# oliverhu/rama

Hardware: AMD Instinct MI355X
Metric: tokens/sec decode + matvec achieved-HBM-GB/s vs roofline, llama2-7B fp32 1xMI355X (higher is better)
Workload: dtype f32

## Files before the change

rama_amd/csrc/chain.hpp:

```cpp
#pragma once
#define RAMA_CHAIN_HPP 1
#include "kernels.hpp"
#include "chain_params.hpp"
#include "ref_order.hpp"
#include "topp_sort.hpp"
#include "seqsum_fast.hpp"
#include "handoff.hpp"

namespace rama {


template <int NW>
struct SeqSumShared {
    Inc w[2][NW];
    int ev[2][NW];
    int pos[2];
    float cum[2];
};

template <int R, int NW>
__device__ __forceinline__ void seqsum_round(const float* a, int n, SeqSumShared<NW>& sh, int par) {
    RAMA_NO_CONTRACT
    const int tid = threadIdx.x, lane = tid & 63, wave = tid >> 6;
    const int pos = sh.pos[par];
// ... 328 lines not shown
    float v[R];
#pragma unroll
    for (int k = 0; k < R; k++) { const int i = (int)threadIdx.x * R + k; const float t = a[scan_slot(min(i, n - 1))]; v[k] = i < n ? t : 0.0f; }
    const int nreal = min(max((n - (int)threadIdx.x * R + 7) >> 3, 0), R / 8);
    return seq_sum_fast<NW, R>(v, fs, out, nreal);
}
template <int NW>
__device__ __forceinline__ bool seq_sum_lds_fast(const float* a, int n, FastSumShared<NW>& fs, float* out) {
    const int per = (n + 64 * NW - 1) / (64 * NW);
    if (n < kFastSumMin || per > 64) return false;
    seq_sum_fast_prepare<NW>(fs);
    if (per <= 8) return seq_sum_lds_fast_r<NW, 8>(a, n, fs, out);
    if (per <= 16) return seq_sum_lds_fast_r<NW, 16>(a, n, fs, out);
    if (per <= 32) return seq_sum_lds_fast_r<NW, 32>(a, n, fs, out);
    return seq_sum_lds_fast_r<NW, 64>(a, n, fs, out);
}
template <int NW>
__device__ __forceinline__ float seq_sum_cascade(const float* a, int n, FastSumShared<NW>& fsn, PredShared<NW>& ps, SeqSumShared<NW>& sh) {
    float sum;
    if (!seq_sum_lds_fast<NW>(a, n, fsn, &sum)) { __syncthreads(); if (!seq_sum_predict<NW>(a, n, ps, &sum)) sum = seq_sum_exact<NW>(a, n, sh); }
    return sum;
}
__global__ __launch_bounds__(kNormThreads) void rmsnorm_chain_kernel(float* o, const float* x, const float* w, int n, float* copy_to, int stride = 0) {
    RAMA_NO_CONTRACT
    o += (size_t)blockIdx.x * stride; x += (size_t)blockIdx.x * stride;
    extern __shared__ __attribute__((aligned(16))) float s_sq[];
    __shared__ SeqSumShared<kNormWaves> sh;
    __shared__ PredShared<kNormWaves> ps;
    __shared__ FastSumShared<kNormWaves> fsn;
    const int tid = threadIdx.x;
    SEQ_STAMP(0);
    const bool vec = n % 4 == 0 && ((((uintptr_t)x | (uintptr_t)w | (uintptr_t)o | (uintptr_t)copy_to) & 15) == 0) && n <= 16 * kNormThreads;
    if (vec) {
        const int n4 = n >> 2;
        f4 xv[4], wv[4];
#pragma unroll
        for (int k = 0; k < 4; k++) xv[k] = reinterpret_cast<const f4*>(x)[min(tid + kNormThreads * k, n4 - 1)];
#pragma unroll
        for (int k = 0; k < 4; k++) wv[k] = reinterpret_cast<const f4*>(w)[min(tid + kNormThreads * k, n4 - 1)];
#pragma unroll
        for (int k = 0; k < 4; k++) {
            const int i = tid + kNormThreads * k;
            if (i < n4) {
                float* d = s_sq + scan_slot(4 * i);
                d[0] = xv[k].x * xv[k].x; d[1] = xv[k].y * xv[k].y; d[2] = xv[k].z * xv[k].z; d[3] = xv[k].w * xv[k].w;
            }
        }
        __syncthreads();
        float ss;
        if (!seq_sum_lds_fast<kNormWaves>(s_sq, n, fsn, &ss)) { __syncthreads(); if (!seq_sum_predict<kNormWaves>(s_sq, n, ps, &ss)) ss = seq_sum_exact<kNormWaves>(s_sq, n, sh); }
        const float v = 1.0f / sqrtf(ss / (float)n + 1e-5f);
#pragma unroll
        for (int k = 0; k < 4; k++) {
            const int i = tid + kNormThreads * k;
            if (i < n4) {
                if (copy_to) reinterpret_cast<f4*>(copy_to)[i] = xv[k];
                f4 r;
                r.x = wv[k].x * (v * xv[k].x); r.y = wv[k].y * (v * xv[k].y); r.z = wv[k].z * (v * xv[k].z); r.w = wv[k].w * (v * xv[k].w);
                reinterpret_cast<f4*>(o)[i] = r;
            }
        }
        SEQ_STAMP(6);
        return;
    }
    for (int i = tid; i < n; i += kNormThreads) { const float a = x[i]; s_sq[scan_slot(i)] = a * a; }
    __syncthreads();
    float ss;
    if (!seq_sum_lds_fast<kNormWaves>(s_sq, n, fsn, &ss)) { __syncthreads(); if (!seq_sum_predict<kNormWaves>(s_sq, n, ps, &ss)) ss = seq_sum_exact<kNormWaves>(s_sq, n, sh); }
    const float v = 1.0f / sqrtf(ss / (float)n + 1e-5f);
    for (int i = tid; i < n; i += kNormThreads) {
        const float a = x[i];
        if (copy_to) copy_to[i] = a;
        o[i] = w[i] * (v * a);
    }
}

__global__ __launch_bounds__(kNormThreads) void softmax_chain_kernel(float* x, int n) {
    RAMA_NO_CONTRACT
    extern __shared__ __attribute__((aligned(16))) float s_e[];
    __shared__ SeqSumShared<kNormWaves> sh;
    __shared__ PredShared<kNormWaves> ps;
    __shared__ FastSumShared<kNormWaves> fsn;
    __shared__ float red[16];
    __shared__ unsigned long long s_tab[32];
    const int tid = threadIdx.x;
    exp_tab_fill(s_tab);
    float mx = -INFINITY;
    for (int i = tid; i < n; i += kNormThreads) mx = fmaxf(mx, x[i]);
    mx = block_max(mx, red);
    for (int i = tid; i < n; i += kNormThreads) s_e[scan_slot(i)] = expf_glibc_tab(x[i] - mx, s_tab);
    __syncthreads();
    const float sum = seq_sum_cascade<kNormWaves>(s_e, n, fsn, ps, sh);
    for (int i = tid; i < n; i += kNormThreads) x[i] = s_e[scan_slot(i)] / sum;
}


__device__ __forceinline__ __amdgpu_buffer_rsrc_t make_rsrc_uniform(const void* p, unsigned bytes) {
    const unsigned long long b = (unsigned long long)(uintptr_t)p;
    const unsigned lo = __builtin_amdgcn_readfirstlane((unsigned)b), hi = __builtin_amdgcn_readfirstlane((unsigned)(b >> 32));
    return make_rsrc(reinterpret_cast<const void*>((uintptr_t)(((unsigned long long)hi << 32) | lo)), (unsigned)__builtin_amdgcn_readfirstlane((int)bytes));
}
__device__ __forceinline__ f4 ld_nt_s(__amdgpu_buffer_rsrc_t r, unsigned voff, unsigned soff) {
    return __builtin_bit_cast(f4, __builtin_amdgcn_raw_buffer_load_b128(r, (int)voff, (int)soff, 2));
}

#ifdef RAMA_CHAIN_STAMPS
__device__ unsigned long long g_chain_stamps[64];
__device__ unsigned long long g_chain_all[3 * 4096];
#define CHAIN_STAMP(id) do { if (threadIdx.x == 0) { const unsigned long long t_ = __builtin_amdgcn_s_memrealtime(); \
        if (blockIdx.x == RAMA_CHAIN_STAMP_BLOCK) g_chain_stamps[id] = t_; \
        if (blockIdx.x < 4096 && ((id) == 0 || (id) == 2 || (id) == 4)) g_chain_all[3 * blockIdx.x + (id) / 2] = t_; } } while (0)
#else
#define CHAIN_STAMP(id) do { } while (0)
#endif

constexpr unsigned long long kLeadErr = 0x3100ull;
template <int W, int D, int XD, int EPI, int NORM = CNORM_NONE, int LR = 64>
__device__ __forceinline__ void gemv_chain_body(const ChainParams p, int bid_in) {
    RAMA_NO_CONTRACT
    CHAIN_STAMP(0);
    static_assert(D % XD == 0, "the x ring must divide the weight ring");
    extern __shared__ __attribute__((aligned(16))) float xs[];
    __shared__ float relay[64];
    constexpr int WL = W;
    const int lane = threadIdx.x & 63;
    const int wave_all = WL == 1 ? 0 : __builtin_amdgcn_readfirstlane(threadIdx.x >> 6);
    const int wave = wave_all;
    const int j = lane & 3, rr = lane >> 2;
    const int groups = (p.rows + 15) >> 4;
    if constexpr (NORM == CNORM_LEAD) {
        if (bid_in == 0) {
#ifndef RAMA_LEAD_SOLO
#define RAMA_LEAD_SOLO 1
#endif
            constexpr bool SOLO = RAMA_LEAD_SOLO && WL > 1 && LR * WL <= 64;
            constexpr int WD = SOLO ? 1 : WL, LD = SOLO ? LR * WL : LR;
            if (SOLO && wave_all != 0) return;
            FastSumShared<WD>& fs = *reinterpret_cast<FastSumShared<WD>*>(xs);
#ifdef RAMA_CHAIN_STAMPS
            if (threadIdx.x == 0) g_chain_stamps[40] = __builtin_amdgcn_s_memrealtime();
#endif
            const unsigned ep = *p.epoch;
            const __amdgpu_buffer_rsrc_t rxl = make_rsrc_uniform(p.x, (unsigned)p.K * 4u);
            seq_sum_fast_prepare<WD>(fs);
            float a[LD];
#pragma unroll
            for (int u = 0; u < LD / 4; u++) {
                const f4 xv = ld_c(rxl, ((unsigned)threadIdx.x * (unsigned)LD + 4u * (unsigned)u) * 4u);
                a[4 * u] = xv.x * xv.x; a[4 * u + 1] = xv.y * xv.y; a[4 * u + 2] = xv.z * xv.z; a[4 * u + 3] = xv.w * xv.w;
            }
#ifdef RAMA_CHAIN_STAMPS
            { float t_ = 0.0f;
#pragma unroll
              for (int k = 0; k < LD; k++) t_ += a[k];
              asm volatile("" :: "v"(t_)); }
            if (threadIdx.x == 0) g_chain_stamps[41] = __builtin_amdgcn_s_memrealtime();
#endif
            float ss;
            if (!seq_sum_fast<WD, LD>(a, fs, &ss)) {
                __syncthreads();
#pragma unroll
                for (int k = 0; k < LD; k++) { const int i = (int)threadIdx.x * LD + k; if (i < p.K) xs[i] = a[k]; }
                __syncthreads();
                if (threadIdx.x == 0) { float s_ = 0.0f; for (int i = 0; i < p.K; i++) s_ = s_ + xs[i]; xs[p.K] = s_; }
                __syncthreads();
                ss = xs[p.K];
            }
            const float v = 1.0f / sqrtf(ss / (float)p.K + 1e-5f);
            if (threadIdx.x == 0) put_tagged(p.lead, v, ep);
#ifdef RAMA_CHAIN_STAMPS
            if (threadIdx.x == 0) g_chain_stamps[42] = __builtin_amdgcn_s_memrealtime();
#endif
            if (p.xout) {
                for (int i = threadIdx.x; i < p.K; i += WD * 64) p.xout[i] = p.nw[i] * (v * p.x[i]);
            }
            return;
        }
    }
    const int bid = NORM == CNORM_LEAD ? bid_in - 1 : bid_in;
    int half = -1, bid_g = bid;
    if (W == 1 && p.half_from > 0 && bid >= p.half_from) { half = (bid - p.half_from) & 1; bid_g = p.half_from + ((bid - p.half_from) >> 1); }
    const int m = __builtin_amdgcn_readfirstlane(bid_g / groups), g = __builtin_amdgcn_readfirstlane(bid_g - m * groups);
    const float* Wm = m == 0 ? p.w[0] : (m == 1 ? p.w[1] : p.w[2]);
    const int nblk = p.K >> 4;
    const int nchunk = (nblk + D - 1) / D;
    const bool lane_ok = half < 0 || lane < 32;
    const unsigned lane16 = half < 0 ? (unsigned)lane * 16u : (lane < 32 ? (unsigned)half * 512u + (unsigned)lane * 16u : kOOB);
    static_assert(D % 16 == 0, "a chunk is made of whole 16-block stretches");
    const int n16 = (nblk + 15) >> 4;
    auto stretch = [&](int q) {
        const int left = min(max(nblk - q * 16, 0), 16);
        return make_rsrc_uniform(Wm + ((size_t)g * (size_t)nblk + (size_t)min(q, n16) * 16) * 256, (unsigned)left * 1024u);
    };
    unsigned vo[4];
#pragma unroll
    for (int k = 0; k < 4; k++) vo[k] = lane16 + (unsigned)k * 4096u;
    const __amdgpu_buffer_rsrc_t rx = make_rsrc_uniform(p.x, (unsigned)p.K * 4u);
    const int n4 = p.K >> 2;
    constexpr int T = WL * 64, XU = 16;
    f4 xa[XU];
#pragma unroll
    for (int u = 0; u < XU; u++) xa[u] = ld_c(rx, ((int)threadIdx.x + T * u) < n4 ? (unsigned)((int)threadIdx.x + T * u) * 16u : kOOB);
    f4 ga[NORM != CNORM_NONE ? XU : 1];
    if constexpr (NORM != CNORM_NONE) {
        const __amdgpu_buffer_rsrc_t rg = make_rsrc_uniform(p.nw, (unsigned)p.K * 4u);
#pragma unroll
        for (int u = 0; u < XU; u++) ga[u] = ld_c(rg, ((int)threadIdx.x + T * u) < n4 ? (unsigned)((int)threadIdx.x + T * u) * 16u : kOOB);
    }
    f4 wr[D];
#pragma unroll
    for (int h = 0; h < D / 16; h++) {
        const __amdgpu_buffer_rsrc_t r0 = stretch(wave * (D / 16) + h);
#pragma unroll
        for (int u = 0; u < 16; u++) wr[h * 16 + u] = ld_nt(r0, vo[u >> 2] + (unsigned)(u & 3) * 1024u);
    }
    const int row = lane_ok ? 16 * g + (half > 0 ? 8 : 0) + rr : p.rows + 16;
    float xold = 0.0f, rc = 1.0f, rs = 0.0f;
    unsigned long long tabv = 0;
    int pos = 0;
    if (EPI == CEPI_RESID) {
        if (j == 0 && row < p.rows) xold = p.resid[row];
    } else if (EPI == CEPI_SWIGLU) {
        tabv = kExp2fTab[lane & 31];
    } else if (EPI == CEPI_QKV) {
        pos = p.ctl ? p.ctl->pos : p.pos_val;
        if (m < 2) {
            const int i = ((row & ~1) % p.head_size) >> 1;
            rc = p.fr[(size_t)pos * (p.head_size >> 1) + i];
            rs = p.fi[(size_t)pos * (p.head_size >> 1) + i];
        }
    }
    CHAIN_STAMP(1);
    if constexpr (NORM == CNORM_TREE) {
        float ssl = 0.0f;
#pragma unroll
        for (int u = 0; u < XU; u++) ssl = ssl + ((xa[u].x * xa[u].x + xa[u].y * xa[u].y) + (xa[u].z * xa[u].z + xa[u].w * xa[u].w));
        ssl = wave_sum(ssl);
        if (W > 1) {
            __shared__ float wss[W];
            if (lane == 0) wss[wave] = ssl;
            __syncthreads();
            ssl = wss[0];
#pragma unroll
            for (int w_ = 1; w_ < W; w_++) ssl = ssl + wss[w_];
        }
        const float v = 1.0f / sqrtf(ssl / (float)p.K + 1e-5f);
#pragma unroll
        for (int u = 0; u < XU; u++) {
            xa[u].x = ga[u].x * (v * xa[u].x); xa[u].y = ga[u].y * (v * xa[u].y);
            xa[u].z = ga[u].z * (v * xa[u].z); xa[u].w = ga[u].w * (v * xa[u].w);
        }
    }
    if constexpr (NORM == CNORM_LEAD) {
        float v = 0.0f;
        {
            const unsigned ep = *p.epoch;
            unsigned long long word = 0;
            long spins = 0;
            while (true) {
                if (lane == 0) word = __hip_atomic_load(p.lead, __ATOMIC_RELAXED, __HIP_MEMORY_SCOPE_AGENT);
                word = ((unsigned long long)(unsigned)__builtin_amdgcn_readfirstlane((int)(word >> 32)) << 32) | (unsigned)__builtin_amdgcn_readfirstlane((int)(unsigned)word);
                if ((unsigned)(word >> 32) == ep) break;
                __builtin_amdgcn_s_sleep(1);
                ++spins;
                if ((spins & 255) == 0 && __hip_atomic_load(p.err, __ATOMIC_RELAXED, __HIP_MEMORY_SCOPE_AGENT)) break;
                if (spins > (1L << 22)) { if (lane == 0) __hip_atomic_store(p.err, kLeadErr, __ATOMIC_RELAXED, __HIP_MEMORY_SCOPE_AGENT); break; }
            }
            v = __uint_as_float((unsigned)word);
        }
        CHAIN_STAMP(5);
#pragma unroll
        for (int u = 0; u < XU; u++) {
            xa[u].x = ga[u].x * (v * xa[u].x); xa[u].y = ga[u].y * (v * xa[u].y);
            xa[u].z = ga[u].z * (v * xa[u].z); xa[u].w = ga[u].w * (v * xa[u].w);
        }
    }
    if constexpr (NORM == CNORM_EXACT) {
        __shared__ PredShared<W> nps;
        float* sq = xs + p.K + chain_pad_floats(W, D, XD);
#pragma unroll
        for (int u = 0; u < XU; u++) {
            const int i = (int)threadIdx.x + T * u;
            if (i < n4) {
                float* d = sq + scan_slot(4 * i);
                d[0] = xa[u].x * xa[u].x; d[1] = xa[u].y * xa[u].y; d[2] = xa[u].z * xa[u].z; d[3] = xa[u].w * xa[u].w;
            }
        }
        __syncthreads();
        const float ss = seq_sum_ripples<W>(sq, p.K, nps);
        const float v = 1.0f / sqrtf(ss / (float)p.K + 1e-5f);
#pragma unroll
        for (int u = 0; u < XU; u++) {
            xa[u].x = ga[u].x * (v * xa[u].x); xa[u].y = ga[u].y * (v * xa[u].y);
            xa[u].z = ga[u].z * (v * xa[u].z); xa[u].w = ga[u].w * (v * xa[u].w);
        }
    }
    {
#pragma unroll
        for (int u = 0; u < XU; u++) {
            const int i = (int)threadIdx.x + T * u;
            float* d = xs + (i < n4 ? 16 * (i >> 2) + (i & 3) : p.K);
            d[0] = xa[u].x; d[4] = xa[u].y; d[8] = xa[u].z; d[12] = xa[u].w;
        }
        for (int i0 = (int)threadIdx.x + T * XU; i0 < n4; i0 += T * 8) {
            f4 a[8];
#pragma unroll
            for (int u = 0; u < 8; u++) a[u] = ld_c(rx, (i0 + T * u) < n4 ? (unsigned)(i0 + T * u) * 16u : kOOB);
#pragma unroll
            for (int u = 0; u < 8; u++) {
                const int i = i0 + T * u;
                float* d = xs + (i < n4 ? 16 * (i >> 2) + (i & 3) : p.K);
                d[0] = a[u].x; d[4] = a[u].y; d[8] = a[u].z; d[12] = a[u].w;
            }
        }
    }
    for (int i = p.K + (int)threadIdx.x; i < p.K + chain_pad_floats(W, D, XD); i += T) xs[i] = 0.0f;
    __syncthreads();
    CHAIN_STAMP(2);
    const f4* xq = reinterpret_cast<const f4*>(xs) + j;
    float v = 0.0f;
    if (W == 1) {
        f4 xr[XD];
#pragma unroll
        for (int u = 0; u < XD; u++) xr[u] = xq[4 * u];
        for (int c = 0; c < nchunk; c++) {
            __amdgpu_buffer_rsrc_t rn[D / 16];
#pragma unroll
            for (int h = 0; h < D / 16; h++) rn[h] = stretch((c + 1) * (D / 16) + h);
            const f4* xc = xq + 4 * c * D;
#pragma unroll
            for (int u = 0; u < D; u++) {
                const f4 xv = xr[u % XD];
                xr[u % XD] = xc[4 * (u + XD)];
                const f4 wv = wr[u];
                v = v + wv.x * xv.x;
                v = v + wv.y * xv.y;
                v = v + wv.z * xv.z;
                v = v + wv.w * xv.w;
                wr[u] = ld_nt(rn[u >> 4], vo[(u & 15) >> 2] + (unsigned)(u & 3) * 1024u);
                __builtin_amdgcn_sched_barrier(0);
            }
        }
    } else {
        auto premultiply = [&](int c) {
            const f4* xc = xq + 4 * c * D;
#pragma unroll
            for (int u = 0; u < D; u++) {
                const f4 xv = xc[4 * u];
                wr[u].x = wr[u].x * xv.x; wr[u].y = wr[u].y * xv.y; wr[u].z = wr[u].z * xv.z; wr[u].w = wr[u].w * xv.w;
                if constexpr (D > 16) { if ((u & 7) == 7) __builtin_amdgcn_sched_barrier(0); }
            }
        };
        if (wave == 0) premultiply(0);
        CHAIN_STAMP(3);
        for (int c = 0; c < nchunk; c++) {
            if ((c % W) == wave) {
                if (c < 24) CHAIN_STAMP(8 + 2 * c);
                if (c > 0) v = relay[lane];
                __amdgpu_buffer_rsrc_t rn[D / 16];
#pragma unroll
                for (int h = 0; h < D / 16; h++) rn[h] = stretch((c + W) * (D / 16) + h);
#pragma unroll
                for (int u = 0; u < D; u++) {
                    const f4 pv = wr[u];
                    v = v + pv.x;
                    v = v + pv.y;
                    v = v + pv.z;
                    v = v + pv.w;
                    wr[u] = ld_nt(rn[u >> 4], vo[(u & 15) >> 2] + (unsigned)(u & 3) * 1024u);
                    __builtin_amdgcn_sched_barrier(0);
                }
                if (c + 1 < nchunk) relay[lane] = v;
                if (c < 24) CHAIN_STAMP(9 + 2 * c);
            } else if (((c + 1) % W) == wave && c + 1 < nchunk) {
                premultiply(c + 1);
            }
            __syncthreads();
        }
    }
    CHAIN_STAMP(4);
    if (W > 1 && ((nchunk - 1) % W) != wave) return;
    float d;
    if (p.lane_reduce == LANES_STRIDED) {
        const float t2 = v + dpp_mov<0x4E>(v);
        d = t2 + dpp_mov<0xB1>(t2);
    } else if (p.lane_reduce == LANES_SEQUENTIAL) {
        d = ((dpp_mov<0x00>(v) + dpp_mov<0x55>(v)) + dpp_mov<0xAA>(v)) + dpp_mov<0xFF>(v);
    } else {
        const float t2 = v + dpp_mov<0xB1>(v);
        d = t2 + dpp_mov<0x4E>(t2);
    }
    if (EPI == CEPI_STORE) {
        if (j == 0 && row < p.rows) { float* o = m == 0 ? p.o[0] : (m == 1 ? p.o[1] : p.o[2]); o[row] = d; }
    } else if (EPI == CEPI_RESID) {
        if (j == 0 && row < p.rows) { p.o[0][row] = d; p.resid[row] = xold + d; }
    } else if (EPI == CEPI_QKV) {
        const float other = __shfl_xor(d, 4);
        const float a = (rr & 1) ? other : d, b = (rr & 1) ? d : other;
        float out = d;
        if (m < 2) out = (rr & 1) ? a * rs + b * rc : a * rc - b * rs;
        if (j == 0 && row < p.rows) {
            float* o = m == 0 ? p.o[0] : (m == 1 ? p.o[1] : p.o[2]);
            o[row] = out;
            if (m == 1) p.kc[(size_t)pos * p.rows + row] = out;
            else if (m == 2) p.vc[(size_t)pos * p.rows + row] = out;
        }
    } else {
        const float h3 = __shfl_xor(d, 4);
        __shared__ unsigned long long s_tab[32];
        s_tab[lane & 31] = tabv;
        __builtin_amdgcn_wave_barrier();
        if (j == 0 && !(rr & 1) && row < p.rows) {
            const float sl = d * (1.0f / (1.0f + expf_glibc_tab(-d, s_tab)));
            p.o[0][row >> 1] = sl * h3;
            p.o[1][row >> 1] = h3;
        }
    }
}

template <int W, int D, int XD, int EPI, int NORM = CNORM_NONE, int LR = 64, int TAG = 0>
__global__ __launch_bounds__(W * 64) void gemv_chain_kernel(ChainParams p) {
    gemv_chain_body<W, D, XD, EPI, NORM, LR>(p, (int)blockIdx.x);
}


template <int I>
__device__ __forceinline__ float mul_row(float a, float w) {
    float r;
    if (I == 0) asm("v_mul_f32_dpp %0, %1, %2 row_newbcast:0 row_mask:0xf bank_mask:0xf" : "=v"(r) : "v"(a), "v"(w));
    else if (I == 1) asm("v_mul_f32_dpp %0, %1, %2 row_newbcast:1 row_mask:0xf bank_mask:0xf" : "=v"(r) : "v"(a), "v"(w));
    else if (I == 2) asm("v_mul_f32_dpp %0, %1, %2 row_newbcast:2 row_mask:0xf bank_mask:0xf" : "=v"(r) : "v"(a), "v"(w));
    else asm("v_mul_f32_dpp %0, %1, %2 row_newbcast:3 row_mask:0xf bank_mask:0xf" : "=v"(r) : "v"(a), "v"(w));
    return r;
}

template <int TPW, int EPI>
__global__ __launch_bounds__(kGcThreads) void gemm_chain_kernel(GemmChainParams p) {
    RAMA_NO_CONTRACT
    constexpr int T = kGcWaves * TPW;
    constexpr int WN = kGcBlocks * 64 / kGcThreads;
    constexpr int PPT = kGcBlocks * 4;
    constexpr int XF = (T * PPT + kGcThreads - 1) / kGcThreads;
    extern __shared__ __attribute__((aligned(16))) float gsm[];
    f4* wl = reinterpret_cast<f4*>(gsm);
    float* xl = gsm + 2 * kGcBlocks * 256;
    const int tid = threadIdx.x, lane = tid & 63;
    const int wave = __builtin_amdgcn_readfirstlane(tid >> 6);
    const int groups = (p.rows + 15) >> 4;
    const int m = __builtin_amdgcn_readfirstlane(blockIdx.x / groups), g = blockIdx.x - m * groups;
    const float* Wm = m == 0 ? p.w[0] : (m == 1 ? p.w[1] : p.w[2]);
    const int nblk = p.K >> 4;
    const int nchunk = (nblk + kGcBlocks - 1) / kGcBlocks;
    const __amdgpu_buffer_rsrc_t rx = make_rsrc_uniform(p.x, (unsigned)((size_t)p.n_tok * (size_t)p.xstride * 4u));
    f4 wreg[kGcSets][WN], xreg[kGcSets][XF];

    auto issue = [&](int c, f4 (&wr)[WN], f4 (&xr)[XF]) {
        const int left = min(max(nblk - c * kGcBlocks, 0), kGcBlocks);
        const __amdgpu_buffer_rsrc_t rw = make_rsrc_uniform(Wm + ((size_t)g * (size_t)nblk + (size_t)min(c, nchunk) * kGcBlocks) * 256, (unsigned)left * 1024u);
#pragma unroll
        for (int n = 0; n < WN; n++) wr[n] = ld_nt(rw, (unsigned)(tid + kGcThreads * n) * 16u);
#pragma unroll
        for (int n = 0; n < XF; n++) {
            const int q = tid + kGcThreads * n, t = q / PPT, i = q % PPT;
            const int k = c * (kGcBlocks * 16) + i * 4;
            xr[n] = ld_c(rx, (t < p.n_tok && k < p.K) ? (unsigned)(((size_t)t * (size_t)p.xstride + (size_t)k) * 4u) : kOOB);
        }
    };
    auto stage = [&](int slot, const f4 (&wr)[WN], const f4 (&xr)[XF]) {
#pragma unroll
        for (int n = 0; n < WN; n++) wl[slot * (kGcBlocks * 64) + tid + kGcThreads * n] = wr[n];
#pragma unroll
        for (int n = 0; n < XF; n++) {
            const int q = tid + kGcThreads * n, t = q / PPT, i = q % PPT;
            if (T * PPT % kGcThreads == 0 || q < T * PPT) {
                float* d = xl + ((size_t)slot * T + t) * (kGcBlocks * 16) + 16 * (i >> 2) + (i & 3);
                d[0] = xr[n].x; d[4] = xr[n].y; d[8] = xr[n].z; d[12] = xr[n].w;
            }
        }
    };
    const int jj = lane >> 4, r16 = lane & 15;
    typedef float f2 __attribute__((ext_vector_type(2)));
    float acc1 = 0.0f;
    f2 acc2[TPW >= 2 ? TPW / 2 : 1];
#pragma unroll
    for (int tp = 0; tp < (TPW >= 2 ? TPW / 2 : 1); tp++) acc2[tp] = f2{0.0f, 0.0f};
    auto compute = [&](int slot) {
        const f4* wq = wl + slot * (kGcBlocks * 64) + (r16 * 4 + jj);
        const float* xb = xl + ((size_t)slot * T + (size_t)wave * TPW) * (kGcBlocks * 16) + 4 * jj + (r16 & 3);
        f4 w0, w1;
        float xa[TPW], xc[TPW];
        auto fetch = [&](int u, f4& wv, float (&xv)[TPW]) {
            wv = wq[u * 64];
#pragma unroll
            for (int tt = 0; tt < TPW; tt++) xv[tt] = xb[tt * (kGcBlocks * 16) + 16 * u];
        };
        auto sums = [&](const f4& wv, const float (&xs1)[TPW]) {
            if constexpr (TPW == 1) {
                float v = acc1;
                v = v + mul_row<0>(xs1[0], wv.x);
                v = v + mul_row<1>(xs1[0], wv.y);
                v = v + mul_row<2>(xs1[0], wv.z);
                v = v + mul_row<3>(xs1[0], wv.w);
                acc1 = v;
            } else {
#pragma unroll
                for (int tp = 0; tp < TPW / 2; tp++) {
                    f2 v = acc2[tp];
                    v = v + f2{mul_row<0>(xs1[2 * tp], wv.x), mul_row<0>(xs1[2 * tp + 1], wv.x)};
                    v = v + f2{mul_row<1>(xs1[2 * tp], wv.y), mul_row<1>(xs1[2 * tp + 1], wv.y)};
                    v = v + f2{mul_row<2>(xs1[2 * tp], wv.z), mul_row<2>(xs1[2 * tp + 1], wv.z)};
                    v = v + f2{mul_row<3>(xs1[2 * tp], wv.w), mul_row<3>(xs1[2 * tp + 1], wv.w)};
                    acc2[tp] = v;
                }
            }
            if constexpr (TPW == 1) asm volatile("" : "+v"(acc1));
            else {
#pragma unroll
                for (int tp = 0; tp < TPW / 2; tp++) asm volatile("" : "+v"(acc2[tp]));
            }
        };
        fetch(0, w0, xa);
#pragma unroll
        for (int u = 0; u < kGcBlocks; u += 2) {
            fetch(u + 1, w1, xc);
            __builtin_amdgcn_sched_barrier(0);
            sums(w0, xa);
            __builtin_amdgcn_sched_barrier(0);
            if (u + 2 < kGcBlocks) fetch(u + 2, w0, xa);
            __builtin_amdgcn_sched_barrier(0);
            sums(w1, xc);
            __builtin_amdgcn_sched_barrier(0);
        }
    };
    issue(0, wreg[0], xreg[0]);
    issue(1, wreg[1], xreg[1]);
    stage(0, wreg[0], xreg[0]);
    issue(2, wreg[0], xreg[0]);
    __syncthreads();
#pragma unroll 1
    for (int c = 0; c < nchunk; c += 2) {
        stage(1, wreg[1], xreg[1]);
        __builtin_amdgcn_sched_barrier(0);
        issue(c + 3, wreg[1], xreg[1]);
        __builtin_amdgcn_sched_barrier(0);
        compute(0);
        __syncthreads();
        stage(0, wreg[0], xreg[0]);
        __builtin_amdgcn_sched_barrier(0);
        issue(c + 4, wreg[0], xreg[0]);
        __builtin_amdgcn_sched_barrier(0);
        compute(1);
        __syncthreads();
    }
    const int row = 16 * g + r16;
#pragma unroll
    for (int tt = 0; tt < TPW; tt++) {
        const int t = wave * TPW + tt;
        const float v = TPW == 1 ? acc1 : acc2[tt / 2][tt & 1];
        float d;
        if (p.lane_reduce == LANES_STRIDED) {
            const float t2 = v + __shfl_xor(v, 32);
            d = t2 + __shfl_xor(t2, 16);
        } else if (p.lane_reduce == LANES_SEQUENTIAL) {
            const int l16 = (int)(threadIdx.x & 15);
            d = ((__shfl(v, l16) + __shfl(v, l16 + 16)) + __shfl(v, l16 + 32)) + __shfl(v, l16 + 48);
        } else {
            const float t2 = v + __shfl_xor(v, 16);
            d = t2 + __shfl_xor(t2, 32);
        }
        const float other = __shfl_xor(d, 1);
        if (t >= p.n_tok) continue;
        if (EPI == CEPI_STORE) {
            if (jj == 0 && row < p.rows) p.o[0][(size_t)t * p.ostride + row] = d;
        } else if (EPI == CEPI_RESID) {
            if (jj == 0 && row < p.rows) {
                if (p.o[0]) p.o[0][(size_t)t * p.ostride + row] = d;
                float* xr_ = p.resid + (size_t)t * p.rstride + row;
                *xr_ = *xr_ + d;
            }
        } else if (EPI == CEPI_QKV) {
            const int pos = p.seqs ? p.seqs[t].pos : p.pos0 + t;
            float* kcl = p.seqs ? p.seqs[t].kc + p.layer_off : p.kc;
            float* vcl = p.seqs ? p.seqs[t].vc + p.layer_off : p.vc;
            float out = d;
            if (m < 2) {
                const int i = ((row & ~1) % p.head_size) >> 1;
                const float rc = p.fr[(size_t)pos * (p.head_size >> 1) + i], rs = p.fi[(size_t)pos * (p.head_size >> 1) + i];
                const float a = (r16 & 1) ? other : d, b = (r16 & 1) ? d : other;
                out = (r16 & 1) ? a * rs + b * rc : a * rc - b * rs;
            }
            if (jj == 0 && row < p.rows) {
                if (m == 0) p.o[0][(size_t)t * p.ostride + row] = out;
                else if (m == 1) kcl[(size_t)pos * p.rows + row] = out;
                else vcl[(size_t)pos * p.rows + row] = out;
            }
        } else {
            if (jj == 0 && !(r16 & 1) && row < p.rows) {
                const float sl = d * (1.0f / (1.0f + expf_glibc(-d)));
                p.o[0][(size_t)t * p.ostride + (row >> 1)] = sl * other;
            }
        }
    }
}


typedef const __attribute__((address_space(1))) f4* gf4p;
__device__ __forceinline__ gf4p gptr4(const float* p) { return (gf4p)reinterpret_cast<const f4*>(p); }
template <int NW>
__device__ __forceinline__ void attention_chain_body(RefAttnParams p, int h, int y, int lds_seq) {
    RAMA_NO_CONTRACT
    constexpr int T = NW * 64;
    extern __shared__ __attribute__((aligned(16))) float sm[];
    __shared__ SeqSumShared<NW> sh;
    __shared__ PredShared<NW> ps;
    __shared__ FastSumShared<NW> fsn;
    __shared__ float red[16];
    __shared__ unsigned long long s_tab[32];
    const int tid = threadIdx.x, lane = tid & 63;
    const int wave = __builtin_amdgcn_readfirstlane(tid >> 6);
    exp_tab_fill(s_tab);
    const int pos = p.seqs ? p.seqs[y].pos : (p.ctl ? p.ctl->pos : p.pos_val) + y;
    if (p.seqs) { p.kc = p.seqs[y].kc + p.layer_off; p.vc = p.seqs[y].vc + p.layer_off; }
    p.q += (size_t)y * p.tok_stride; p.xb += (size_t)y * p.tok_stride;
    if (p.att) p.att += (size_t)y * p.att_stride;
    const int hs = p.head_size, hs4 = hs >> 2;
    float* s_q = sm;
    float* s_p = sm + ((hs + 3) & ~3);
    float* s_att = s_p + ((lds_seq + 3) & ~3);
    const int region_off = (((hs + 3) & ~3) + ((lds_seq + 3) & ~3) + lds_seq + (lds_seq >> 5) + 4 + 3) & ~3;
    float* region = sm + region_off;
    const size_t col = (size_t)h * hs;
    SEQ_STAMP(8);
    for (int i = tid; i < hs; i += T) s_q[i] = p.q[col + i];
    constexpr int U = NW >= 16 ? 4 : 8;
    const int tile4 = kAttTile * hs4;
    int er[U], ec[U];
#pragma unroll
    for (int u = 0; u < U; u++) { const int e = tid + u * T; er[u] = e / hs4; ec[u] = e - er[u] * hs4; }
    auto vissue = [&](int t0, f4 (&vr)[U]) {
#pragma unroll
        for (int u = 0; u < U; u++) {
            const int tr = min(t0 + er[u], pos), c4 = ec[u];
            vr[u] = __builtin_nontemporal_load(gptr4(p.vc + (size_t)tr * p.dim + col) + c4);
        }
    };
// ... 509 lines not shown
```

Baseline: 206.4.

## Stream x staging into LDS interleaved with matvec chunks for single-wave no-norm path

For the W==1, no-norm chain variant, the bulk copy of the input vector into shared memory is removed from the prologue. Instead, slices of x are loaded and written to LDS progressively while earlier chunks of the dot product run, with wavefront fences and barriers between slices. The aim is to shorten the serial startup before weight streaming begins and to overlap x staging with weight loads. The cost is added control flow and a dependence on ordering guarantees, since each chunk must only read x slices that have already been written.

Result: faster. 208.6 (median of 6 runs) (+1.1%).

```diff
diff --git a/rama_amd/csrc/chain.hpp b/rama_amd/csrc/chain.hpp
--- a/rama_amd/csrc/chain.hpp
+++ b/rama_amd/csrc/chain.hpp
@@ -654,15 +654,17 @@
             float* d = xs + (i < n4 ? 16 * (i >> 2) + (i & 3) : p.K);
             d[0] = xa[u].x; d[4] = xa[u].y; d[8] = xa[u].z; d[12] = xa[u].w;
         }
-        for (int i0 = (int)threadIdx.x + T * XU; i0 < n4; i0 += T * 8) {
-            f4 a[8];
-#pragma unroll
-            for (int u = 0; u < 8; u++) a[u] = ld_c(rx, (i0 + T * u) < n4 ? (unsigned)(i0 + T * u) * 16u : kOOB);
-#pragma unroll
-            for (int u = 0; u < 8; u++) {
-                const int i = i0 + T * u;
-                float* d = xs + (i < n4 ? 16 * (i >> 2) + (i & 3) : p.K);
-                d[0] = a[u].x; d[4] = a[u].y; d[8] = a[u].z; d[12] = a[u].w;
+        if constexpr (!(W == 1 && NORM == CNORM_NONE)) {
+            for (int i0 = (int)threadIdx.x + T * XU; i0 < n4; i0 += T * 8) {
+                f4 a[8];
+#pragma unroll
+                for (int u = 0; u < 8; u++) a[u] = ld_c(rx, (i0 + T * u) < n4 ? (unsigned)(i0 + T * u) * 16u : kOOB);
+#pragma unroll
+                for (int u = 0; u < 8; u++) {
+                    const int i = i0 + T * u;
+                    float* d = xs + (i < n4 ? 16 * (i >> 2) + (i & 3) : p.K);
+                    d[0] = a[u].x; d[4] = a[u].y; d[8] = a[u].z; d[12] = a[u].w;
+                }
             }
         }
     }
@@ -675,7 +677,7 @@
         f4 xr[XD];
 #pragma unroll
         for (int u = 0; u < XD; u++) xr[u] = xq[4 * u];
-        for (int c = 0; c < nchunk; c++) {
+        auto chunk = [&](int c) __attribute__((always_inline)) {
             __amdgpu_buffer_rsrc_t rn[D / 16];
 #pragma unroll
             for (int h = 0; h < D / 16; h++) rn[h] = stretch((c + 1) * (D / 16) + h);
@@ -692,7 +694,35 @@
                 wr[u] = ld_nt(rn[u >> 4], vo[(u & 15) >> 2] + (unsigned)(u & 3) * 1024u);
                 __builtin_amdgcn_sched_barrier(0);
             }
-        }
+        };
+        int c = 0;
+        if constexpr (NORM == CNORM_NONE) {
+            constexpr int XN = D >= 32 ? XU : XU / 2;
+            static_assert(4 * XN >= D && 4 * XU >= D + XD, "a trip runs at least its peeled chunk");
+#pragma unroll 1
+            for (int s4 = T * XU; s4 < n4; s4 += T * XN) {
+                f4 xn[XN];
+#pragma unroll
+                for (int u = 0; u < XN; u++) {
+                    const int i = s4 + lane + T * u;
+                    xn[u] = ld_c(rx, i < n4 ? (unsigned)i * 16u : kOOB);
+                }
+                const int cl = ((s4 >> 2) - XD) / D;
+                chunk(c++);
+#pragma unroll 1
+                for (; c < cl; c++) chunk(c);
+#pragma unroll
+                for (int u = 0; u < XN; u++) {
+                    const int i = s4 + lane + T * u;
+                    float* d = xs + (i < n4 ? 16 * (i >> 2) + (i & 3) : p.K);
+                    d[0] = xn[u].x; d[4] = xn[u].y; d[8] = xn[u].z; d[12] = xn[u].w;
+                }
+                __builtin_amdgcn_fence(__ATOMIC_RELEASE, "wavefront");
+                __builtin_amdgcn_wave_barrier();
+            }
+        }
+#pragma unroll 1
+        for (; c < nchunk; c++) chunk(c);
     } else {
         auto premultiply = [&](int c) {
             const f4* xc = xq + 4 * c * D;
```
